# Plachtaa/FAcodec

Hardware: NVIDIA H100
Metric: audio_seconds_per_second (higher is better)
Workload: dtype f32 I/O and accumulation; every product is a 3-MMA split of fp32 operands: fp16 hi + 2^11-scaled fp16 lo (22 mantissa bits, register-promoted accumulation) upstream of the VQ, bf16 hi + bf16 lo (16 bits) downstream

## Files before the change

### facodec_b200/csrc/conv_tc.cu

```cuda
#include <cuda_bf16.h>
#include <cuda_fp16.h>

#include <cstring>
#include <mutex>
#include <type_traits>

#include "common.cuh"
#include "conv_tc_common.cuh"
#include "kernels.h"

namespace fac {

namespace {

using namespace tc;

enum Prec { P_TF32 = 0, P_BF16 = 1, P_F16S = 2, P_F16X2 = 3, P_NONE = -1 };

template <int P> struct PrecT {
    static constexpr int KG = P == P_TF32 ? 4 : 2;
    static constexpr int planes = P == P_F16S ? 1 : 2;
    static constexpr int ksteps = P == P_TF32 ? 2 : 1;
    static constexpr int kind = P == P_TF32 ? WG_TF32 : (P == P_BF16 ? WG_BF16 : WG_F16);
};

__host__ __device__ constexpr int prec_kg(int P) { return P == P_TF32 ? 4 : 2; }
__host__ __device__ constexpr int prec_planes(int P) { return P == P_F16S ? 1 : 2; }
__host__ __device__ constexpr uint32_t master_bytes(bool promoted, int nchunk, int promote_every, int ni) {
    return promoted && nchunk > promote_every ? (uint32_t)ni / 2 * 4 * kThreads : 0u;
}

template <int NI>
__device__ __forceinline__ void zero_acc(float (&a)[NI / 2]) {
#pragma unroll
    for (int i = 0; i < NI / 2; ++i) a[i] = 0.f;
}

template <int P, int NI>
__device__ __forceinline__ void mma_pass(float (&acc)[NI / 2], uint32_t a_addr, uint32_t a_lbo, uint32_t b_addr,
                                         uint32_t b_lbo) {
#pragma unroll
    for (int ks = 0; ks < PrecT<P>::ksteps; ++ks)
        wgmma_ss<NI, PrecT<P>::kind>(acc, gdesc(a_addr + ks * 2 * a_lbo, a_lbo, 128), gdesc(b_addr + ks * 2 * b_lbo, b_lbo, 128));
}

struct Tile {
    int row0, col0, nw;
    int warp, lane;
};

template <int NI, int GROUP = NI, typename F>
__device__ __forceinline__ void for_each_pair(const Tile& tl, const float (&acc)[NI / 2], F&& f) {
#pragma unroll
    for (int j = 0; j < NI / 8; ++j) {
        if (j > 0 && (8 * j) % GROUP == 0 && 8 * j >= tl.nw) break;
#pragma unroll
        for (int h = 0; h < 2; ++h) {
            const int row = tl.row0 + 16 * tl.warp + (tl.lane >> 2) + 8 * h;
            const int col = tl.col0 + 8 * j + 2 * (tl.lane & 3);
            f(row, col, acc[4 * j + 2 * h], acc[4 * j + 2 * h + 1]);
        }
    }
}

template <bool FAST>
__device__ __forceinline__ float act_out(int act, float v, float al, float ia) {
    if (act == ACT_SNAKE) return FAST ? fmaf(ia, sin2_mufu(al * v), v) : snake_fast(v, al, ia);
    if (act == ACT_TANH) return tanhf(v);
    if (act == ACT_MISH) return mish_f(v);
    return v;
}

template <int P1, int P2, bool TT>
constexpr bool groupable() { return P1 != P_F16S && P2 == P_NONE && !TT; }

template <int P1, int P2, bool PROMO, int NI, int MINB, bool TT, bool C2D>
__device__ __forceinline__ void conv_tc_body(const TcConvParams& p) {
    constexpr bool FUSED = P2 != P_NONE;
    constexpr bool GROUPABLE = groupable<P1, P2, TT>() && !C2D;
    static_assert(!C2D || (P1 == P_F16X2 && PROMO && !FUSED && !TT), "2-D taps: the promoted fp16 hi + scaled-lo class only");
    static_assert(!TT || (NI == 64 && !FUSED), "transposed tiles: <= 64 channels x 64 time steps per warpgroup");
    static_assert(NI % 16 == 0 && NI <= (PROMO || MINB == 2 ? 64 : (P1 == P_F16S ? 256 : 128)),
                  "accumulator registers: <= 64 / 128 columns (256 in the one-pass fp16 class at one CTA per SM)");
    constexpr bool F16X2 = P1 == P_F16X2;
    constexpr bool DEC = P1 == P_BF16 || P1 == P_F16S;
    using T1 = PrecT<P1>;
    extern __shared__ __align__(1024) uint8_t smem[];
    uint64_t* full = reinterpret_cast<uint64_t*>(smem);

    const int tid = threadIdx.x, wg = tid >> 7;
    const int BM = 64 * p.MT;
    const int N = p.N, NW = p.MT == 2 ? N : N / 2;
    Tile tl;
    tl.row0 = p.MT == 2 ? 64 * wg : 0;
    tl.col0 = p.MT == 2 ? 0 : wg * NW;
    tl.nw = NW;
    tl.warp = (tid >> 5) & 3;
    tl.lane = tid & 31;
    const int t0 = blockIdx.x * BM, ntile = blockIdx.y, b = blockIdx.z;
    const int Kr = p.Kr, dil = p.dil, Rpad = p.Rpad, nchunk = p.nchunk, S = p.stagesB;
    const int G = GROUPABLE ? p.group : 1;
    const int R = BM + (C2D ? 2 * p.row2d + 2 : (Kr - 1) * dil);
    const int nstep1 = G == 4 ? nchunk >> 2 : (G == 2 ? nchunk >> 1 : nchunk);
    const uint32_t a_plane = (uint32_t)G * T1::KG * Rpad * 16, a_bytes = a_plane * T1::planes;
    uint8_t* abuf = smem + kSmemHdr;
    float4* master = reinterpret_cast<float4*>(abuf + 2 * (size_t)a_bytes);
    const uint32_t m_bytes = master_bytes(PROMO, nchunk, p.promote_every, NI);
    uint8_t* wbuf = abuf + 2 * (size_t)a_bytes + m_bytes;
    uint8_t* a2buf = m_bytes ? reinterpret_cast<uint8_t*>(master) : wbuf + (size_t)S * p.b_slot;
    const uint32_t w_unit1 = (uint32_t)Kr * T1::planes * T1::KG * N * 16;
    const uint32_t w_unit2 = FUSED ? (uint32_t)prec_planes(P2) * prec_kg(P2) * N * 16 : 0;
    const int units = nstep1 + (FUSED ? p.nchunk2 : 0);

    if (tid == 0) {
        for (int i = 0; i < S; ++i) mbar_init(&full[i], 1);
        fence_mbar_init();
    }
    __syncthreads();
    auto issue_w = [&](int u) {
        uint64_t* bar = &full[u % S];
        uint8_t* dst = wbuf + (size_t)(u % S) * p.b_slot;
        const uint8_t* src;
        uint32_t bytes;
        if (u < nstep1) {
            src = reinterpret_cast<const uint8_t*>(p.wblob) + ((size_t)ntile * nchunk + (size_t)u * G) * w_unit1;
            bytes = G * w_unit1;
        } else { src = reinterpret_cast<const uint8_t*>(p.wblob2) + (size_t)(u - nstep1) * w_unit2; bytes = w_unit2; }
        mbar_arrive_expect_tx(bar, bytes);
        bulk_g2s(dst, src, bytes, bar);
    };
    if (tid == 0)
        for (int u = 0; u < S - 1 && u < units; ++u) issue_w(u);

    const PadMap pm = PadMap::lane(p.lane_len, b, p.Tin, p.pad_left_s, p.pad_right_s, p.reflect);
    const float* __restrict__ xb = p.x + (size_t)b * p.x_bstride;
    auto produce = [&](int s) {
        uint8_t* ahi = abuf + (size_t)(s & 1) * a_bytes;
        auto run = [&](auto grouped) {
            constexpr bool GR = decltype(grouped)::value;
            const int c = GR ? s * G : s;
            if constexpr (P1 == P_TF32) produce_chunk<kThreads, GR, false>(p, pm, xb, c, G, t0, R, Rpad, ahi, ahi + a_plane, tid);
            else if constexpr (P1 == P_BF16) produce_chunk<kThreads, GR, true>(p, pm, xb, c, G, t0, R, Rpad, ahi, ahi + a_plane, tid);
            else if constexpr (P1 == P_F16S) produce_chunk<kThreads, GR, true, 4, false, false, true>(p, pm, xb, c, G, t0, R, Rpad, ahi, ahi, tid);
            else produce_chunk<kThreads, GR, false, 4, false, true>(p, pm, xb, c, G, t0, R, Rpad, ahi, ahi + a_plane, tid);
        };
        if constexpr (GROUPABLE) {
            if (G > 1) run(std::true_type());
            else run(std::false_type());
        } else {
            run(std::false_type());
        }
        fence_proxy_async();
    };
    produce(0);

    float acc[NI / 2];
    float crs[F16X2 ? NI / 2 : 1];
    zero_acc<NI>(acc);
    if constexpr (F16X2) zero_acc<NI>(crs);
    const uint32_t a_lbo = (uint32_t)Rpad * 16, b_lbo = (uint32_t)N * 16;
    const uint32_t abase = smem_u32(abuf), wbase = smem_u32(wbuf), a2base = smem_u32(a2buf);
    const int BM2 = BM;

    auto promote = [&](bool first, bool last) {
        if constexpr (PROMO) {
#pragma unroll
            for (int q = 0; q < NI / 8; ++q) {
                float w[4];
#pragma unroll
                for (int e = 0; e < 4; ++e) {
                    const int i = 4 * q + e;
                    if constexpr (F16X2) { w[e] = acc[i] + crs[i] * kLoUnscale; crs[i] = 0.f; }
                    else w[e] = acc[i];
                }
                float4 m = first ? make_float4(0.f, 0.f, 0.f, 0.f) : master[q * kThreads + tid];
                m.x += w[0]; m.y += w[1]; m.z += w[2]; m.w += w[3];
                if (!last) master[q * kThreads + tid] = m;
                acc[4 * q + 0] = last ? m.x : 0.f;
                acc[4 * q + 1] = last ? m.y : 0.f;
                acc[4 * q + 2] = last ? m.z : 0.f;
                acc[4 * q + 3] = last ? m.w : 0.f;
            }
        }
    };

#pragma unroll 1
    for (int u = 0; u < units; ++u) {
        __syncthreads();
        if (tid == 0 && u + S - 1 < units) issue_w(u + S - 1);
        mbar_wait(&full[u % S], (uint32_t)(u / S) & 1u);
        const uint32_t wslot = wbase + (uint32_t)(u % S) * p.b_slot;
        wg_fence();
        if (u < nstep1) {
            const uint32_t a0 = abase + (uint32_t)(u & 1) * a_bytes + (uint32_t)tl.row0 * 16;
            const uint32_t b0 = wslot + (uint32_t)tl.col0 * 16;
            auto mma_tap = [&](uint32_t ahi, uint32_t bhi) {
                const uint32_t alo = ahi + a_plane, blo = bhi + T1::KG * b_lbo;
                if constexpr (TT) {
                    mma_pass<P1, NI>(acc, bhi, b_lbo, ahi, a_lbo);
                    mma_pass<P1, NI>(crs, bhi, b_lbo, alo, a_lbo);
                    mma_pass<P1, NI>(crs, blo, b_lbo, ahi, a_lbo);
                } else if constexpr (P1 == P_F16S) {
                    mma_pass<P1, NI>(acc, ahi, a_lbo, bhi, b_lbo);
                } else if constexpr (F16X2) {
                    mma_pass<P1, NI>(acc, ahi, a_lbo, bhi, b_lbo);
                    mma_pass<P1, NI>(crs, ahi, a_lbo, blo, b_lbo);
                    mma_pass<P1, NI>(crs, alo, a_lbo, bhi, b_lbo);
                } else {
                    mma_pass<P1, NI>(acc, ahi, a_lbo, bhi, b_lbo);
                    mma_pass<P1, NI>(acc, ahi, a_lbo, blo, b_lbo);
// ... 105 lines not shown
    for_each_pair<NI>(tl, acc, [&](int row, int col, float v0, float v1) {
        const int t = t0 + row;
        if (t >= p.Tout) return;
        if constexpr (C2D) {
            const float2 bi = __ldg(reinterpret_cast<const float2*>(bi_p + col));
            v0 += bi.x; v1 += bi.y;
            if (act == ACT_LRELU) { v0 = v0 >= 0.f ? v0 : 0.01f * v0; v1 = v1 >= 0.f ? v1 : 0.01f * v1; }
            if (rb) { const float2 r = *reinterpret_cast<const float2*>(rb + (size_t)t * p.ldy + col); v0 += r.x; v1 += r.y; }
            const int f = t % p.row2d;
            if (f == 0 || f == p.row2d - 1) { v0 = 0.f; v1 = 0.f; }
            *reinterpret_cast<float2*>(yb + (size_t)t * p.ldy + col) = make_float2(v0, v1);
            return;
        }
        if (bi_p) { const float2 bi = __ldg(reinterpret_cast<const float2*>(bi_p + col)); v0 += bi.x; v1 += bi.y; }
        if (act == ACT_SNAKE) {
            const float2 al = __ldg(reinterpret_cast<const float2*>(al_p + col));
            const float2 ia = __ldg(reinterpret_cast<const float2*>(ia_p + col));
            v0 = act_out<DEC>(ACT_SNAKE, v0, al.x, ia.x);
            v1 = act_out<DEC>(ACT_SNAKE, v1, al.y, ia.y);
        } else if (act != ACT_NONE) {
            v0 = act_out<DEC>(act, v0, 0.f, 0.f);
            v1 = act_out<DEC>(act, v1, 0.f, 0.f);
        }
        if (rb) { const float2 r = *reinterpret_cast<const float2*>(rb + (size_t)t * p.ldy + col); v0 += r.x; v1 += r.y; }
        *reinterpret_cast<float2*>(yb + (size_t)t * p.ldy + col) = make_float2(v0, v1);
    });
}

template <int P1, int P2, bool PROMO, int NI, int MINB = 1, bool TT = false>
__global__ void __launch_bounds__(kThreads, groupable<P1, P2, TT>() && NI <= 128 ? 2 : MINB) conv_tc_kernel(TcConvParams p) {
    conv_tc_body<P1, P2, PROMO, NI, MINB, TT, false>(p);
}

template <int NI>
__global__ void __launch_bounds__(kThreads, 2) conv2d_tc_kernel(TcConvParams p) {
    conv_tc_body<P_F16X2, P_NONE, true, NI, 2, false, true>(p);
}

}

namespace {
constexpr size_t kSmemCap = 227 * 1024;
constexpr size_t kSmemCap2 = 113 * 1024;
int plan_prec(const TcConvParams& p) {
    return p.g1f16 ? P_F16S : (p.f16x2 ? P_F16X2 : (p.bf16 ? P_BF16 : P_TF32));
}
constexpr int f16s_wide_nw(bool fused) { return fused ? 192 : 256; }
}

bool tc_conv_plan(TcConvParams& p) {
    if ((p.Cin % 4) != 0 || ((p.Cin * p.vf) % kChunk) != 0 || (p.Cout % 16) != 0) return false;
    if (p.bf16 && p.promoted) return false;
    if (p.f16x2 && !p.promoted) return false;
    if (p.g1f16 && !p.bf16) return false;
    if (p.tt && !p.f16x2) return false;
    if (p.row2d && (p.Kr != 9 || p.vf != 1 || !p.f16x2 || p.tt || p.fused || p.row2d < 3)) return false;
    if (p.fused && ((p.promoted && (!p.f16x2 || p.tt)) || p.Cin != p.Cout || p.vf != 1 || p.Cout > 256)) return false;
    const int P1 = plan_prec(p), P2 = p.fused ? (p.f16x2 ? P_F16X2 : (p.bf16 ? P_BF16 : P_TF32)) : P_NONE;
    p.nchunk = p.Cin * p.vf / kChunk;
    p.nchunk2 = p.fused ? p.Cout / kChunk : 0;
    p.promote_every = p.promoted ? (p.f16x2 ? (48 / p.Kr < 1 ? 1 : 48 / p.Kr) : (8 / p.Kr < 1 ? 1 : 8 / p.Kr)) : 1;
    if (p.fused && p.promoted && p.nchunk2 > 48) return false;
    const int nw_max = p.promoted ? 64 : 128;
    constexpr size_t kAReserve = 40 * 1024;
    int N = 0;
    for (int cand = p.fused ? p.Cout : 256; cand >= 16 && N == 0; cand -= 16) {
// ... 26 lines not shown
        return l;
    };
    auto group = [&](int S, int MT, size_t cap) {
        if (p.Kr > 3 || p.tt || p.fused || p.g1f16) return 1;
        for (int G = 4; G > 1; G /= 2)
            if (G <= p.max_group && p.nchunk % G == 0 && (!p.promoted || p.promote_every % G == 0) && layout(S, MT, G).total <= cap) return G;
        return 1;
    };
    const bool unit2 = p.fused && p.promoted;
    const bool want2 = p.promoted ? !p.tt : (p.occ2_maxn > 0 && N <= p.occ2_maxn);
    for (int two = want2 ? 1 : 0; two >= (unit2 ? 1 : 0); --two) {
        const size_t cap = two ? kSmemCap2 : kSmemCap;
        const int nwl = two ? 64 : nw_max;
        for (int S = 2; S >= 1; --S)
            for (int MT = 2; MT >= 1; --MT) {
                const int NW = MT == 2 ? N : N / 2;
                const bool wide = !two && P1 == P_F16S && NW == f16s_wide_nw(p.fused);
                if ((NW > nwl && !wide) || NW % 16 || (unit2 && NW != 64)) continue;
                if (wide && layout(2, 1, 1).total <= kSmemCap2) continue;
                const Layout l1 = layout(S, MT, 1);
                if (l1.total > cap) continue;
                const int G = group(S, MT, l1.total <= kSmemCap2 ? kSmemCap2 : cap);
                const Layout l = layout(S, MT, G);
                p.N = N; p.MT = MT; p.Rpad = l.Rpad; p.R2pad = 64 * MT; p.stagesB = S; p.b_slot = (int)l.slot;
                p.group = G;
                p.smem_bytes = l.total;
                p.occ2 = two;
                return true;
            }
    }
    return false;
}

size_t tc_blob_floats(const TcConvParams& p) {
    if (p.g1f16) return (size_t)(p.Cout / p.N) * p.nchunk * p.Kr * 2 * p.N * 4;
    return (size_t)(p.Cout / p.N) * p.nchunk * p.Kr * 2 * ((p.bf16 || p.f16x2) ? 2 : 4) * p.N * 4;
}

static inline uint16_t bf16_rn_host(float f) {
    uint32_t u;
    memcpy(&u, &f, 4);
    u += 0x7FFFu + ((u >> 16) & 1u);
    return (uint16_t)(u >> 16);
}

void tc_pack_blob(const TcConvParams& p, const float* wp, int ldw, float* blob) {
    const int Cw = p.Cin * p.vf;
    if (p.g1f16) {
        uint16_t* ob = reinterpret_cast<uint16_t*>(blob);
        size_t o16 = 0;
        for (int nt = 0; nt < p.Cout / p.N; ++nt)
            for (int c = 0; c < p.nchunk; ++c)
                for (int tap = 0; tap < p.Kr; ++tap)
                    for (int k8 = 0; k8 < 2; ++k8)
                        for (int n = 0; n < p.N; ++n)
                            for (int e = 0; e < 8; ++e) {
                                int kk = tap * Cw + c * tc::kChunk + k8 * 8 + e;
                                __half v = __float2half_rn(wp[(size_t)kk * ldw + nt * p.N + n]);
                                uint16_t bits;
                                memcpy(&bits, &v, 2);
                                ob[o16++] = bits;
                            }
        return;
    }
    if (p.f16x2) {
        uint16_t* ob = reinterpret_cast<uint16_t*>(blob);
// ... 31 lines not shown
                                    uint32_t hu = (uint32_t)hi << 16;
                                    float hf;
                                    memcpy(&hf, &hu, 4);
                                    ob[o16++] = hl == 0 ? hi : bf16_rn_host(w - hf);
                                }
        return;
    }
    size_t o = 0;
    for (int nt = 0; nt < p.Cout / p.N; ++nt)
        for (int c = 0; c < p.nchunk; ++c)
            for (int tap = 0; tap < p.Kr; ++tap)
                for (int hl = 0; hl < 2; ++hl)
                    for (int k4 = 0; k4 < 4; ++k4)
                        for (int n = 0; n < p.N; ++n)
                            for (int e = 0; e < 4; ++e) {
                                int kk = tap * Cw + c * tc::kChunk + k4 * 4 + e;
                                float w = wp[(size_t)kk * ldw + nt * p.N + n];
                                uint32_t u;
                                memcpy(&u, &w, 4);
                                uint32_t hu = (u + 0x1000u) & 0xFFFFE000u;
                                float hi;
                                memcpy(&hi, &hu, 4);
                                float lo = w - hi;
                                uint32_t lu;
                                memcpy(&lu, &lo, 4);
                                lu = (lu + 0x1000u) & 0xFFFFE000u;
                                float lo_r;
                                memcpy(&lo_r, &lu, 4);
                                blob[o++] = hl == 0 ? hi : lo_r;
                            }
}

namespace {
template <int P1, int P2, bool PROMO, int NI, int MINB = 1, bool TT = false, bool C2D = false>
cudaError_t launch_one(const TcConvParams& p, dim3 grid, cudaStream_t st) {
    auto* kern = [] {
        if constexpr (C2D) return conv2d_tc_kernel<NI>;
        else return conv_tc_kernel<P1, P2, PROMO, NI, MINB, TT>;
    }();
    static bool done[64] = {};
    static std::mutex mu;
    int dev = 0;
    cudaError_t e = cudaGetDevice(&dev);
    if (e != cudaSuccess) return e;
    if (dev < 0 || dev >= 64) return cudaErrorInvalidDevice;
    {
        std::lock_guard<std::mutex> lk(mu);
        if (!done[dev]) {
            e = cudaFuncSetAttribute(kern, cudaFuncAttributeMaxDynamicSharedMemorySize, (int)kSmemCap);
            if (e != cudaSuccess) return e;
            done[dev] = true;
        }
    }
    kern<<<grid, kThreads, p.smem_bytes, st>>>(p);
    return cudaGetLastError();
}
template <int P1, int P2, bool PROMO, int MINB = 1, int NI = (PROMO || MINB == 2 ? 64 : 128), bool C2D = false>
cudaError_t launch_nw(const TcConvParams& p, dim3 grid, cudaStream_t st) {
    const int NW = p.MT == 2 ? p.N : p.N / 2;
    if (NW == NI) return launch_one<P1, P2, PROMO, NI, MINB, false, C2D>(p, grid, st);
    if constexpr (NI > 16) return launch_nw<P1, P2, PROMO, MINB, NI - 16, C2D>(p, grid, st);
    else return cudaErrorInvalidValue;
}
template <int P1, int P2>
cudaError_t launch_occ(const TcConvParams& p, dim3 grid, cudaStream_t st) {
    if (p.occ2) return launch_nw<P1, P2, false, 2>(p, grid, st);
    if constexpr (P1 == P_F16S) {
        constexpr int kWide = f16s_wide_nw(P2 != P_NONE);
        if ((p.MT == 2 ? p.N : p.N / 2) == kWide) return launch_one<P1, P2, false, kWide>(p, grid, st);
    }
    return launch_nw<P1, P2, false, 1>(p, grid, st);
}
}

cudaError_t launch_conv_tc(const TcConvParams& p, cudaStream_t st) {
    if (p.Tout <= 0 || p.B <= 0) return cudaSuccess;
    const int BM = 64 * p.MT;
    dim3 grid((p.Tout + BM - 1) / BM, p.Cout / p.N, p.B);
    if (grid.y > 65535 || grid.z > 65535) return cudaErrorInvalidValue;
    const int P1 = plan_prec(p);
    if (p.row2d) {
        if (P1 != P_F16X2 || !p.promoted || p.fused || p.tt || p.Kr != 9) return cudaErrorInvalidValue;
        return launch_nw<P_F16X2, P_NONE, true, 2, 64, true>(p, grid, st);
    }
    if (p.fused) {
        if (P1 == P_F16X2)
            return (p.MT == 2 ? p.N : p.N / 2) == 64 ? launch_one<P_F16X2, P_F16X2, true, 64, 2>(p, grid, st) : cudaErrorInvalidValue;
        if (P1 == P_F16S) return launch_occ<P_F16S, P_BF16>(p, grid, st);
        if (P1 == P_BF16) return launch_occ<P_BF16, P_BF16>(p, grid, st);
        return launch_occ<P_TF32, P_TF32>(p, grid, st);
    }
    if (p.tt) return launch_one<P_F16X2, P_NONE, true, 64, 1, true>(p, grid, st);
    if (p.promoted)
        return P1 == P_F16X2 ? launch_nw<P_F16X2, P_NONE, true, 2>(p, grid, st) : launch_nw<P_TF32, P_NONE, true, 2>(p, grid, st);
    if (P1 == P_F16S) return launch_occ<P_F16S, P_NONE>(p, grid, st);
    if (P1 == P_BF16) return launch_occ<P_BF16, P_NONE>(p, grid, st);
    return launch_occ<P_TF32, P_NONE>(p, grid, st);
}

}
```

### facodec_b200/csrc/engine.cu

```cuda
#include <cmath>
#include <cstddef>
#include <cstdio>
#include <cstdlib>
#include <cstring>
#include <algorithm>
#include <initializer_list>
#include <map>
#include <memory>
#include <string>
#include <type_traits>
#include <vector>

#include "../../include/facodec_b200.h"
#include "../../include/facodec_b200_debug.h"
#include "common.cuh"
#include "kernels.h"
#include "resample.h"

using namespace fac;

namespace {

constexpr int HOP = 300;
constexpr int LATENT = 1024;
// ... 652 lines not shown

int conv_out_len(int T, int k_eff, int stride) {
    int padding_total = k_eff - stride;
    double n_frames = (double)(T - k_eff + padding_total) / stride + 1.0;
    int ideal = ((int)std::ceil(n_frames) - 1) * stride + (k_eff - padding_total);
    int extra = ideal - T;
    return (T + padding_total + extra - k_eff) / stride + 1;
}
int conv_extra_pad(int T, int k_eff, int stride) {
    int padding_total = k_eff - stride;
    double n_frames = (double)(T - k_eff + padding_total) / stride + 1.0;
    int ideal = ((int)std::ceil(n_frames) - 1) * stride + (k_eff - padding_total);
    return ideal - T;
}

void run_conv(Ctx& c, const ConvW& w, const float* x, float* y, int B, int Tin, int Tout, const ConvOpts& o,
              const char* name) {
    if (c.dry) return;
    if (c.h->use_tc >= (c.vq_critical ? 2 : 1) && w.tc && !o.transposed && !o.valid_len && (o.ldx == 0 || o.ldx == w.Cin) &&
        (o.ldy == 0 || o.ldy == w.Cout) && o.stride == w.vf && (w.vf == 1 || o.dil == 1) && !o.no_bias) {
        TcConvParams tp;
        tp.Cin = w.Cin; tp.Cout = w.Cout; tp.vf = w.vf; tp.Kr = w.Kr; tp.promoted = w.promoted ? 1 : 0;
        tp.dil = w.vf == 1 ? o.dil : 1;
        tp.bf16 = (c.h->dec_bf16 && w.has16 && !w.promoted && !c.vq_critical) ? 1 : 0;
        tp.g1f16 = (tp.bf16 && w.has_f16s && c.h->dec_c7_f16) ? 1 : 0;
        tp.f16x2 = (tp.promoted && c.h->enc_f16 && w.has16) ? 1 : 0;
        tp.occ2_maxn = c.h->tc_occ2;
        tp.Tout = Tout;
        if (tp.f16x2 && c.h->enc_tt) {
            TcConvParams t2 = tp;
            t2.tt = 1;
            if (tc_conv_plan(t2)) tp = t2;
        }
        if (tc_conv_plan(tp)) {
            tp.x = x; tp.y = y; tp.wblob = c.W(tp.g1f16 ? w.tcw_f16s : ((tp.bf16 || tp.f16x2) ? w.tcw16 : w.tcw)); tp.bias = c.W(w.b);
            if (o.in_snake) { tp.in_alpha = c.W(o.in_snake->a); tp.in_inv_alpha = c.W(o.in_snake->ia); }
            tp.out_act = o.act;
            if (o.out_snake) { tp.out_act = ACT_SNAKE; tp.out_alpha = c.W(o.out_snake->a); tp.out_inv_alpha = c.W(o.out_snake->ia); }
            tp.res = o.res;
            tp.B = B; tp.Tin = Tin; tp.ldx = w.Cin;
            tp.PLr = o.pad_left / w.vf;
            tp.pad_left_s = o.pad_left; tp.pad_right_s = o.pad_right; tp.reflect = o.reflect; tp.lane_len = o.lane_len;
            tp.Tout = Tout; tp.ldy = w.Cout;
            tp.x_bstride = (size_t)Tin * w.Cin; tp.y_bstride = (size_t)Tout * w.Cout;
            double flops = 2.0 * B * Tout * (double)w.Cout * w.K * w.Cin;
            double bytes = 4.0 * ((double)B * Tin * w.Cin + (double)B * Tout * w.Cout * (o.res ? 2 : 1) + (double)w.K * w.Cin * w.Cout);
            char det[96];
            snprintf(det, sizeof det, "%s Cin%d Cout%d K%d d%d T%d", name, w.Cin, w.Cout, w.K, o.dil, Tout);
            c.begin(tp.promoted ? "conv_tcp" : "conv_tc", flops, bytes, det);
            c.check(launch_conv_tc(tp, c.st), name);
            c.end();
            return;
        }
    }
    ConvParams p;
    p.x = x; p.y = y;
    p.w = c.W(w.w);
    p.bias = o.no_bias ? nullptr : c.W(w.b);
    if (o.in_snake) { p.in_alpha = c.W(o.in_snake->a); p.in_inv_alpha = c.W(o.in_snake->ia); }
    p.out_act = o.act;
    if (o.out_snake) { p.out_act = ACT_SNAKE; p.out_alpha = c.W(o.out_snake->a); p.out_inv_alpha = c.W(o.out_snake->ia); }
    p.res = o.res; p.valid_len = o.valid_len; p.lane_len = o.lane_len;
    p.B = B; p.Tin = Tin; p.Cin = w.Cin; p.Tout = Tout; p.Cout = w.Cout;
    p.K = w.K; p.dil = o.dil; p.stride = o.stride;
    p.pad_left = o.pad_left; p.pad_right = o.pad_right; p.pad_reflect = o.reflect;
    p.ldw = w.ldw; p.ldy = o.ldy ? o.ldy : w.Cout; p.ldx = o.ldx ? o.ldx : w.Cin;
    p.y_transposed = o.transposed;
// ... 12 lines not shown
          const char* name, bool causal = true) {
    int k_eff = (w.K - 1) * dil + 1;
    o.dil = dil; o.stride = stride;
    const int total = k_eff - stride, extra = conv_extra_pad(T, k_eff, stride);
    o.pad_left = causal ? total : total - total / 2;
    o.pad_right = (causal ? 0 : total / 2) + extra;
    o.reflect = 1;
    int Tout = conv_out_len(T, k_eff, stride);
    run_conv(c, w, x, y, B, T, Tout, o, name);
    return Tout;
}

bool residual_unit_fused(Ctx& c, const ResW& r, const float* x, float* y, int B, int T, bool causal, const int* lane_len) {
    const bool promoted = r.c7.promoted && r.c1.promoted;
    if (!c.h->fuse_res || !r.c7.tc || !r.c1.tc || r.c7.promoted != r.c1.promoted || r.c7.Cin != r.c7.Cout ||
        r.c1.K != 1 || r.c7.vf != 1)
        return false;
    if (c.vq_critical ? (!promoted || c.h->use_tc < 2 || !c.h->enc_f16 || c.h->enc_tt || !r.c7.has16 || !r.c1.has16)
                      : (promoted || c.h->use_tc < 1))
        return false;
    TcConvParams tp;
    tp.Cin = r.c7.Cin; tp.Cout = r.c7.Cout; tp.vf = 1; tp.Kr = r.c7.K; tp.dil = r.dil; tp.fused = 1;
    tp.promoted = promoted ? 1 : 0;
    tp.f16x2 = tp.promoted;
    tp.bf16 = (!promoted && c.h->dec_bf16 && r.c7.has16 && r.c1.has16) ? 1 : 0;
    tp.g1f16 = (tp.bf16 && r.c7.has_f16s && c.h->dec_c7_f16) ? 1 : 0;
    tp.occ2_maxn = c.h->tc_occ2;
    tp.Tout = T;
    if (c.h->fuse_res == 2 && r.c7.Cout > 128) return false;
    if (!tc_conv_plan(tp)) return false;
    TcConvParams q7 = tp, q1 = tp;
    q7.fused = 0; q1.fused = 0; q1.Kr = 1; q1.g1f16 = 0;
    if (!tc_conv_plan(q7) || !tc_conv_plan(q1) || q7.N != tp.N || q1.N != tp.N) return false;
    if (c.dry) return true;
    const int k_eff = (r.c7.K - 1) * r.dil + 1;
    tp.x = x; tp.y = y; tp.res = x;
    tp.wblob = c.W(tp.g1f16 ? r.c7.tcw_f16s : ((tp.bf16 || tp.f16x2) ? r.c7.tcw16 : r.c7.tcw)); tp.bias = c.W(r.c7.b);
    tp.wblob2 = c.W((tp.bf16 || tp.f16x2) ? r.c1.tcw16 : r.c1.tcw); tp.bias2 = c.W(r.c1.b);
    tp.in_alpha = c.W(r.s1.a); tp.in_inv_alpha = c.W(r.s1.ia);
    tp.out_act = ACT_SNAKE; tp.out_alpha = c.W(r.s2.a); tp.out_inv_alpha = c.W(r.s2.ia);
    tp.B = B; tp.Tin = T; tp.ldx = r.c7.Cin;
    const int pl = causal ? k_eff - 1 : (k_eff - 1) - (k_eff - 1) / 2;
    tp.PLr = pl; tp.pad_left_s = pl; tp.pad_right_s = k_eff - 1 - pl; tp.reflect = 1; tp.lane_len = lane_len;
    tp.Tout = T; tp.ldy = r.c7.Cout;
    tp.x_bstride = (size_t)T * r.c7.Cin; tp.y_bstride = (size_t)T * r.c7.Cout;
    double flops = 2.0 * B * T * (double)r.c7.Cout * r.c7.Cin * (r.c7.K + 1);
    double bytes = 4.0 * ((double)B * T * r.c7.Cin * 2 + (double)B * T * r.c7.Cout + (double)(r.c7.K + 1) * r.c7.Cin * r.c7.Cout);
    char det[96];
    snprintf(det, sizeof det, "res.fused C%d K%d d%d T%d", r.c7.Cin, r.c7.K, r.dil, T);
    c.begin(tp.promoted ? "conv_tcp" : "conv_tc", flops, bytes, det);
    c.check(launch_conv_tc(tp, c.st), "res.fused");
    c.end();
    return true;
}

void residual_unit(Ctx& c, const ResW& r, const float* x, float* tmp, float* y, int B, int T, bool causal = true,
                   const int* lane_len = nullptr) {
    if (residual_unit_fused(c, r, x, y, B, T, causal, lane_len)) return;
    ConvOpts o1;
    o1.in_snake = &r.s1;
    o1.out_snake = &r.s2;
    o1.lane_len = lane_len;
    sconv(c, r.c7, x, tmp, B, T, r.dil, 1, o1, "res.conv7", causal);
    ConvOpts o2;
    o2.res = x;
    sconv(c, r.c1, tmp, y, B, T, 1, 1, o2, "res.conv1", causal);
// ... 3681 lines not shown
    cudaSetDevice(h->device);
    cudaStream_t st = (cudaStream_t)stream;
    cudaError_t e = launch_attention(q, k, v, o, B, T, heads, 256, valid_len, st, force_stream ? 1 : 0);
    if (e == cudaSuccess) e = cudaStreamSynchronize(st);
    if (e != cudaSuccess) { h->err = std::string("fac_debug_attention: ") + cudaGetErrorString(e); return FAC_ERR_CUDA; }
    return FAC_OK;
}

int fac_set_option(fac_handle* h, const char* name, int value) {
    if (!h || !name) return FAC_ERR_INVALID;
    if (std::string(name) == "fuse_resunit") { h->fuse_res = value < 0 ? 0 : (value > 2 ? 2 : value); return FAC_OK; }
    if (std::string(name) == "encoder_f16x2") { h->enc_f16 = value != 0; return FAC_OK; }
    if (std::string(name) == "encoder_tt") { h->enc_tt = value != 0; return FAC_OK; }
    if (std::string(name) == "tc_occ2_maxn") { h->tc_occ2 = value < 0 ? 0 : value; return FAC_OK; }
    if (std::string(name) == "decoder_conv7_fp16") { h->dec_c7_f16 = value != 0; return FAC_OK; }
    if (std::string(name) == "overlap_front") { h->overlap_front = value != 0; return FAC_OK; }
    if (std::string(name) == "lstm_v2") { h->lstm_v2 = value != 0; return FAC_OK; }
    if (std::string(name) == "decoder_lstm_fp16") { h->dec_lstm_fp16 = value != 0; return FAC_OK; }
    if (std::string(name) == "attention_stream") { h->attn_stream = value != 0; return FAC_OK; }
    if (std::string(name) == "decoder_bf16") { h->dec_bf16 = value != 0; return FAC_OK; }
    if (std::string(name) == "tensor_cores") { h->use_tc = value < 0 ? 0 : (value > 2 ? 2 : value); return FAC_OK; }
    h->err = std::string("unknown option ") + name;
    return FAC_ERR_INVALID;
}

static int debug_conv_tc(fac_handle* h, const float* x, const float* w_host, const float* bias_host, int B, int Tin, int Cin,
                         int Cout, int K, int dil, int stride, int pad_left, int pad_right, int reflect,
                         const float* in_alpha_host, const float* out_alpha_host, int act, const float* res, float* y,
                         int Tout, int promoted, void* stream, int* group_out, const int* lane_len) {
    if (!h || !x || !w_host || !y) return FAC_ERR_INVALID;
    cudaSetDevice(h->device);
    cudaStream_t st = (cudaStream_t)stream;
    TcConvParams tp;
    tp.Cin = Cin; tp.Cout = Cout; tp.promoted = (promoted == 1 || promoted == 3 || promoted == 4) ? 1 : 0;
    tp.bf16 = (promoted == 2 || promoted == 5) ? 1 : 0;
    tp.f16x2 = (promoted == 3 || promoted == 4) ? 1 : 0;
    tp.tt = promoted == 4 ? 1 : 0;
    tp.g1f16 = promoted == 5 ? 1 : 0;
    tp.occ2_maxn = h->tc_occ2;
    tp.Tout = Tout;
    if (stride == 1) { tp.vf = 1; tp.Kr = K; tp.dil = dil; }
    else if (K == 2 * stride && dil == 1) { tp.vf = stride; tp.Kr = 2; tp.dil = 1; }
    else { h->err = "fac_debug_conv_tc: unsupported stride/kernel"; return FAC_ERR_UNSUPPORTED; }
    if (promoted < 0 || promoted > 5 || !tc_conv_plan(tp)) { h->err = "fac_debug_conv_tc: layer not eligible for the tensor-core path"; return FAC_ERR_UNSUPPORTED; }
    if (group_out) {
        *group_out = tp.group;
        tp.max_group = 1;
        if (!tc_conv_plan(tp)) { h->err = "fac_debug_conv_tc_group1: no one-chunk plan"; return FAC_ERR_UNSUPPORTED; }
    }
    int ldw = (Cout + 3) / 4 * 4;
    std::vector<float> gen((size_t)K * Cin * ldw, 0.f);
    for (int co = 0; co < Cout; ++co)
        for (int ci = 0; ci < Cin; ++ci)
            for (int k = 0; k < K; ++k) gen[((size_t)k * Cin + ci) * ldw + co] = w_host[((size_t)co * Cin + ci) * K + k];
    size_t nb = tc_blob_floats(tp);
    auto al4 = [](size_t v) { return (v + 3) / 4 * 4; };
    size_t o_b = al4(nb), o_ia = al4(o_b + Cout), o_iia = al4(o_ia + Cin), o_oa = al4(o_iia + Cin), o_oia = al4(o_oa + Cout);
    std::vector<float> pk(o_oia + Cout + 16, 0.f);
    tc_pack_blob(tp, gen.data(), ldw, pk.data());
    for (int i = 0; i < Cout; ++i) pk[o_b + i] = bias_host ? bias_host[i] : 0.f;
    for (int i = 0; i < Cin; ++i) { pk[o_ia + i] = in_alpha_host ? in_alpha_host[i] : 1.f; pk[o_iia + i] = 1.0f / (pk[o_ia + i] + 1e-9f); }
    for (int i = 0; i < Cout; ++i) { pk[o_oa + i] = out_alpha_host ? out_alpha_host[i] : 1.f; pk[o_oia + i] = 1.0f / (pk[o_oa + i] + 1e-9f); }
    DevBuf<float> buf;
    const int rc = upload(h, pk, buf, "fac_debug_conv_tc");
    if (rc != FAC_OK) return rc;
    const float* d = buf.get();
    tp.x = x; tp.y = y; tp.wblob = d; tp.bias = d + o_b;
    if (in_alpha_host) { tp.in_alpha = d + o_ia; tp.in_inv_alpha = d + o_iia; }
    tp.out_act = act;
    if (out_alpha_host) { tp.out_act = ACT_SNAKE; tp.out_alpha = d + o_oa; tp.out_inv_alpha = d + o_oia; }
    tp.res = res;
    tp.B = B; tp.Tin = Tin; tp.ldx = Cin;
    tp.PLr = pad_left / tp.vf;
    tp.pad_left_s = pad_left; tp.pad_right_s = pad_right; tp.reflect = reflect; tp.lane_len = lane_len;
    tp.Tout = Tout; tp.ldy = Cout;
    tp.x_bstride = (size_t)Tin * Cin; tp.y_bstride = (size_t)Tout * Cout;
    cudaError_t e = launch_conv_tc(tp, st);
    if (e == cudaSuccess) e = cudaStreamSynchronize(st);
    if (e != cudaSuccess) { h->err = std::string("fac_debug_conv_tc: ") + cudaGetErrorString(e); return FAC_ERR_CUDA; }
    return FAC_OK;
}
// ... 130 lines not shown
    ts["c.weight"] = std::move(t);
    ts["c.bias"] = std::move(b);
    Packer P;
    ConvW c;
    try { c = causal ? pack_convtr(P, ts, "c", stride) : pack_convtr_noncausal(P, ts, "c", stride); }
    catch (const PackError&) { return FAC_ERR_UNSUPPORTED; }
    const long long n = (long long)c.K * Cin * c.Cout;
    if (!out || capacity_floats < n) return n;
    for (int k = 0; k < c.K; ++k)
        for (int ci = 0; ci < Cin; ++ci)
            for (int co = 0; co < c.Cout; ++co) out[((size_t)k * Cin + ci) * c.Cout + co] = P.pack[c.w + ((size_t)k * Cin + ci) * c.ldw + co];
    return n;
}

int fac_debug_pad_map(int L, int pad_left, int pad_right, int reflect, int* out, int n) {
    if (!out || L < 0 || pad_left < 0 || pad_right < 0 || n != pad_left + L + pad_right) return FAC_ERR_INVALID;
    const PadMap pm = PadMap::make(L, pad_left, pad_right, reflect);
    for (int i = 0; i < n; ++i) out[i] = pm.src(i - pad_left);
    return FAC_OK;
}

int fac_debug_lane_pad_map(const int* lane_len, int B, int Tin, int pad_left, int pad_right, int reflect, int* out, int n) {
    if (!out || B <= 0 || Tin < 0 || pad_left < 0 || pad_right < 0 || n != pad_left + Tin + pad_right) return FAC_ERR_INVALID;
    for (int b = 0; lane_len && b < B; ++b)
        if (lane_len[b] < 0 || lane_len[b] > Tin) return FAC_ERR_INVALID;
    for (int b = 0; b < B; ++b) {
        const PadMap pm = PadMap::lane(lane_len, b, Tin, pad_left, pad_right, reflect);
        for (int i = 0; i < n; ++i) out[(size_t)b * n + i] = pm.src(i - pad_left);
    }
    return FAC_OK;
}

static int debug_tc_plan(int Cin, int Cout, int K, int dil, int stride, int Tout, int mode, int occ2_maxn, TcConvParams& tp) {
    if (Cin <= 0 || Cout <= 0 || K <= 0 || dil <= 0 || stride <= 0 || mode < 0 || mode > 9) return FAC_ERR_INVALID;
    tp.Cin = Cin; tp.Cout = Cout; tp.Tout = Tout; tp.occ2_maxn = occ2_maxn;
    tp.promoted = (mode == 1 || mode == 3 || mode == 9) ? 1 : 0;
    tp.bf16 = (mode == 2 || mode == 4 || mode == 7 || mode == 8) ? 1 : 0;
    tp.f16x2 = (mode == 3 || mode == 9) ? 1 : 0;
    tp.fused = (mode == 4 || mode == 5 || mode == 8 || mode == 9) ? 1 : 0;
    tp.g1f16 = (mode == 7 || mode == 8) ? 1 : 0;
    if (mode == 6) { tp.promoted = 1; tp.f16x2 = 1; tp.tt = 1; }
    if (stride == 1) { tp.vf = 1; tp.Kr = K; tp.dil = dil; }
    else if (K == 2 * stride && dil == 1) { tp.vf = stride; tp.Kr = 2; tp.dil = 1; }
    else return FAC_ERR_UNSUPPORTED;
    return tc_conv_plan(tp) ? FAC_OK : FAC_ERR_UNSUPPORTED;
}

int fac_debug_tc_plan(int Cin, int Cout, int K, int dil, int stride, int Tout, int mode, int occ2_maxn, int* out8) {
    if (!out8) return FAC_ERR_INVALID;
    TcConvParams tp;
    const int rc = debug_tc_plan(Cin, Cout, K, dil, stride, Tout, mode, occ2_maxn, tp);
    if (rc != FAC_OK) return rc;
    out8[0] = tp.N; out8[1] = tp.MT; out8[2] = tp.nchunk; out8[3] = tp.stagesB; out8[4] = tp.R2pad;
    out8[5] = (int)tp.smem_bytes; out8[6] = tp.Rpad; out8[7] = tp.promote_every;
    return FAC_OK;
}

int fac_debug_tc_plan_group(int Cin, int Cout, int K, int dil, int stride, int Tout, int mode, int occ2_maxn, int* smem2) {
    TcConvParams tp;
    const int rc = debug_tc_plan(Cin, Cout, K, dil, stride, Tout, mode, occ2_maxn, tp);
    if (rc != FAC_OK) return rc;
    if (smem2) {
        TcConvParams t1 = tp;
        t1.max_group = 1;
        if (!tc_conv_plan(t1)) return FAC_ERR_UNSUPPORTED;
        smem2[0] = (int)tp.smem_bytes;
        smem2[1] = (int)t1.smem_bytes;
    }
    return tp.group;
}

long long fac_debug_tc_pack(const float* w_host, int Cin, int Cout, int K, int stride, int mode, float* blob_out,
                            long long capacity_floats) {
    if (!w_host || Cin <= 0 || Cout <= 0 || K <= 0 || stride <= 0 || mode < 0 || mode > 3) return FAC_ERR_INVALID;
    TcConvParams tp;
    tp.Cin = Cin; tp.Cout = Cout; tp.dil = 1;
    tp.promoted = (mode == 1 || mode == 3) ? 1 : 0; tp.bf16 = mode == 2 ? 1 : 0; tp.f16x2 = mode == 3 ? 1 : 0;
    if (stride == 1) { tp.vf = 1; tp.Kr = K; }
// ... 115 lines not shown
```

### facodec_b200/csrc/kernels.h

```cpp
#pragma once
#include <cuda_runtime.h>
#include <stdint.h>

namespace fac {

struct ConvParams {
    const float* x = nullptr;
    const float* w = nullptr;
    const float* bias = nullptr;
    const float* in_alpha = nullptr;
    const float* in_inv_alpha = nullptr;
    const float* out_alpha = nullptr;
    const float* out_inv_alpha = nullptr;
    const float* res = nullptr;
    const int* valid_len = nullptr;
    const int* lane_len = nullptr;
    float* y = nullptr;
    int B = 0, Tin = 0, Cin = 0, Tout = 0, Cout = 0;
    int K = 1, dil = 1, stride = 1, pad_left = 0, pad_right = 0, pad_reflect = 0;
    int ldw = 0, ldy = 0, ldx = 0;
    int out_act = 0;
    int y_transposed = 0;
    size_t x_bstride = 0, y_bstride = 0;
};
// ... 7 lines not shown
    const float* in_inv_alpha = nullptr;
    const float* out_alpha = nullptr;
    const float* out_inv_alpha = nullptr;
    const float* res = nullptr;
    float* y = nullptr;
    int B = 0, Tin = 0, Cin = 0, ldx = 0;
    int vf = 1;
    int Kr = 1, dil = 1, PLr = 0;
    int pad_left_s = 0, pad_right_s = 0, reflect = 0;
    const int* lane_len = nullptr;
    int Tout = 0, Cout = 0, ldy = 0;
    int out_act = 0;
    int promoted = 0;
    int bf16 = 0;
    int g1f16 = 0;
    int f16x2 = 0;
    int fused = 0;
    int tt = 0;
    int occ2_maxn = 0;
    int max_group = 4;
    const float* wblob2 = nullptr;
    const float* bias2 = nullptr;
    int nchunk2 = 0;
    int promote_every = 1;
    int N = 0, nchunk = 0, Rpad = 0, stagesB = 0;
    int group = 1;
    int MT = 2;
    int b_slot = 0;
    int occ2 = 0;
    int R2pad = 0;
    size_t smem_bytes = 0;
    size_t x_bstride = 0, y_bstride = 0;
    int row2d = 0;
};
bool tc_conv_plan(TcConvParams& p);
size_t tc_blob_floats(const TcConvParams& p);
void tc_pack_blob(const TcConvParams& p, const float* wp, int ldw, float* blob);
cudaError_t launch_conv_tc(const TcConvParams& p, cudaStream_t st);

struct LstmParams {
    const float* xg = nullptr;
    const float* whh_p = nullptr;
    const float* whh_p16 = nullptr;
    int bf16 = 0;
    const uint32_t* whh_p2 = nullptr;
    uint32_t* h16 = nullptr;
    int pass3 = 0;
    uint32_t* state_h = nullptr;
    float* state_c = nullptr;
    const float* skip = nullptr;
    float* y = nullptr;
    float* hT = nullptr;
    unsigned int* bar = nullptr;
    int B = 0, T = 0, H = 0, U = 0, G = 0;
};
struct LstmLaneLens { int len[32]; };
cudaError_t launch_lstm_layer(const LstmParams& p, cudaStream_t st);
cudaError_t launch_lstm2_layer(const LstmParams& p, cudaStream_t st, const LstmLaneLens* lens = nullptr, bool reverse = false);
size_t lstm2_pack_words(int H, int U, int pass3);
void lstm2_pack(const float* whh, int H, int U, int pass3, uint32_t* out);
size_t lstm2_smem_bytes(int H, int U, int pass3);
void lstm2_state_sizes(int H, int U, int pass3, size_t* h_words, size_t* c_floats);
cudaError_t lstm2_read_phase_clocks(long long* out4);
void lstm2_lane_map(int H, int U, int pass3, int b, long long* pos);
constexpr int kLaneMax = 32;
struct LaneCarryParams {
    uint32_t* slot[kLaneMax];
    uint32_t* state_h = nullptr;
// ... 126 lines not shown
```

Baseline: 1052.

## Add four-warpgroup wide kernel for promoted fp16x2 K=7 convs at N=128

New measurement: 1069 (median of 6 runs). 1.02x the previous value.

```diff
diff --git a/facodec_b200/csrc/conv_tc.cu b/facodec_b200/csrc/conv_tc.cu
--- a/facodec_b200/csrc/conv_tc.cu
+++ b/facodec_b200/csrc/conv_tc.cu
@@ -26,9 +26,10 @@
 
 __host__ __device__ constexpr int prec_kg(int P) { return P == P_TF32 ? 4 : 2; }
 __host__ __device__ constexpr int prec_planes(int P) { return P == P_F16S ? 1 : 2; }
-__host__ __device__ constexpr uint32_t master_bytes(bool promoted, int nchunk, int promote_every, int ni) {
-    return promoted && nchunk > promote_every ? (uint32_t)ni / 2 * 4 * kThreads : 0u;
-}
+__host__ __device__ constexpr uint32_t master_bytes(bool promoted, int nchunk, int promote_every, int ni, int threads = kThreads) {
+    return promoted && nchunk > promote_every ? (uint32_t)ni / 2 * 4 * threads : 0u;
+}
+constexpr int kWideThreads = 4 * 128;
 
 template <int NI>
 __device__ __forceinline__ void zero_acc(float (&a)[NI / 2]) {
@@ -74,9 +75,12 @@
 template <int P1, int P2, bool TT>
 constexpr bool groupable() { return P1 != P_F16S && P2 == P_NONE && !TT; }
 
-template <int P1, int P2, bool PROMO, int NI, int MINB, bool TT, bool C2D>
+template <int P1, int P2, bool PROMO, int NI, int MINB, bool TT, bool C2D, int NT = kThreads>
 __device__ __forceinline__ void conv_tc_body(const TcConvParams& p) {
     constexpr bool FUSED = P2 != P_NONE;
+    constexpr bool WIDE = NT == kWideThreads;
+    static_assert(NT == kThreads || (WIDE && P1 == P_F16X2 && PROMO && NI == 64 && !TT && !C2D),
+                  "four warpgroups: the promoted fp16 hi + scaled-lo class at 64 channels per warpgroup only");
     constexpr bool GROUPABLE = groupable<P1, P2, TT>() && !C2D;
     static_assert(!C2D || (P1 == P_F16X2 && PROMO && !FUSED && !TT), "2-D taps: the promoted fp16 hi + scaled-lo class only");
     static_assert(!TT || (NI == 64 && !FUSED), "transposed tiles: <= 64 channels x 64 time steps per warpgroup");
@@ -90,10 +94,10 @@
 
     const int tid = threadIdx.x, wg = tid >> 7;
     const int BM = 64 * p.MT;
-    const int N = p.N, NW = p.MT == 2 ? N : N / 2;
+    const int N = p.N, NW = WIDE ? N / 2 : (p.MT == 2 ? N : N / 2);
     Tile tl;
-    tl.row0 = p.MT == 2 ? 64 * wg : 0;
-    tl.col0 = p.MT == 2 ? 0 : wg * NW;
+    tl.row0 = WIDE ? 64 * (wg & 1) : (p.MT == 2 ? 64 * wg : 0);
+    tl.col0 = WIDE ? (wg >> 1) * NW : (p.MT == 2 ? 0 : wg * NW);
     tl.nw = NW;
     tl.warp = (tid >> 5) & 3;
     tl.lane = tid & 31;
@@ -105,7 +109,7 @@
     const uint32_t a_plane = (uint32_t)G * T1::KG * Rpad * 16, a_bytes = a_plane * T1::planes;
     uint8_t* abuf = smem + kSmemHdr;
     float4* master = reinterpret_cast<float4*>(abuf + 2 * (size_t)a_bytes);
-    const uint32_t m_bytes = master_bytes(PROMO, nchunk, p.promote_every, NI);
+    const uint32_t m_bytes = master_bytes(PROMO, nchunk, p.promote_every, NI, NT);
     uint8_t* wbuf = abuf + 2 * (size_t)a_bytes + m_bytes;
     uint8_t* a2buf = m_bytes ? reinterpret_cast<uint8_t*>(master) : wbuf + (size_t)S * p.b_slot;
     const uint32_t w_unit1 = (uint32_t)Kr * T1::planes * T1::KG * N * 16;
@@ -139,10 +143,10 @@
         auto run = [&](auto grouped) {
             constexpr bool GR = decltype(grouped)::value;
             const int c = GR ? s * G : s;
-            if constexpr (P1 == P_TF32) produce_chunk<kThreads, GR, false>(p, pm, xb, c, G, t0, R, Rpad, ahi, ahi + a_plane, tid);
-            else if constexpr (P1 == P_BF16) produce_chunk<kThreads, GR, true>(p, pm, xb, c, G, t0, R, Rpad, ahi, ahi + a_plane, tid);
-            else if constexpr (P1 == P_F16S) produce_chunk<kThreads, GR, true, 4, false, false, true>(p, pm, xb, c, G, t0, R, Rpad, ahi, ahi, tid);
-            else produce_chunk<kThreads, GR, false, 4, false, true>(p, pm, xb, c, G, t0, R, Rpad, ahi, ahi + a_plane, tid);
+            if constexpr (P1 == P_TF32) produce_chunk<NT, GR, false>(p, pm, xb, c, G, t0, R, Rpad, ahi, ahi + a_plane, tid);
+            else if constexpr (P1 == P_BF16) produce_chunk<NT, GR, true>(p, pm, xb, c, G, t0, R, Rpad, ahi, ahi + a_plane, tid);
+            else if constexpr (P1 == P_F16S) produce_chunk<NT, GR, true, 4, false, false, true>(p, pm, xb, c, G, t0, R, Rpad, ahi, ahi, tid);
+            else produce_chunk<NT, GR, false, 4, false, true>(p, pm, xb, c, G, t0, R, Rpad, ahi, ahi + a_plane, tid);
         };
         if constexpr (GROUPABLE) {
             if (G > 1) run(std::true_type());
@@ -173,9 +177,9 @@
                     if constexpr (F16X2) { w[e] = acc[i] + crs[i] * kLoUnscale; crs[i] = 0.f; }
                     else w[e] = acc[i];
                 }
-                float4 m = first ? make_float4(0.f, 0.f, 0.f, 0.f) : master[q * kThreads + tid];
+                float4 m = first ? make_float4(0.f, 0.f, 0.f, 0.f) : master[q * NT + tid];
                 m.x += w[0]; m.y += w[1]; m.z += w[2]; m.w += w[3];
-                if (!last) master[q * kThreads + tid] = m;
+                if (!last) master[q * NT + tid] = m;
                 acc[4 * q + 0] = last ? m.x : 0.f;
                 acc[4 * q + 1] = last ? m.y : 0.f;
                 acc[4 * q + 2] = last ? m.z : 0.f;
@@ -347,6 +351,11 @@
     conv_tc_body<P1, P2, PROMO, NI, MINB, TT, false>(p);
 }
 
+template <int P2>
+__global__ void __launch_bounds__(kWideThreads, 1) conv_tcp_wide_kernel(TcConvParams p) {
+    conv_tc_body<P_F16X2, P2, true, 64, 1, false, false, kWideThreads>(p);
+}
+
 template <int NI>
 __global__ void __launch_bounds__(kThreads, 2) conv2d_tc_kernel(TcConvParams p) {
     conv_tc_body<P_F16X2, P_NONE, true, NI, 2, false, true>(p);
@@ -439,6 +448,23 @@
     return false;
 }
 
+bool tc_conv_plan_promoted_wide(TcConvParams& p) {
+    if (!p.promoted || !p.f16x2 || p.tt || p.row2d || p.vf != 1 || p.Kr != 7) return false;
+    TcConvParams q = p;
+    if (!tc_conv_plan(q) || q.N != 128) return false;
+    constexpr int BM = 128, S = 2, kPieces = 2 * 2;
+    int Rpad = BM + (q.Kr - 1) * q.dil;
+    while (Rpad % 8 != 2) ++Rpad;
+    const size_t a_bytes = (size_t)kPieces * Rpad * 16, slot = (size_t)q.Kr * kPieces * q.N * 16;
+    const size_t master = master_bytes(true, q.nchunk, q.promote_every, q.N / 2, kWideThreads);
+    const size_t total = kSmemHdr + 2 * a_bytes + master + S * slot;
+    if (total > kSmemCap || (q.fused && (size_t)kPieces * q.nchunk2 * BM * 16 > master)) return false;
+    q.MT = 2; q.Rpad = Rpad; q.R2pad = BM; q.stagesB = S; q.b_slot = (int)slot; q.group = 1;
+    q.smem_bytes = total; q.occ2 = 0; q.wide = 1;
+    p = q;
+    return true;
+}
+
 size_t tc_blob_floats(const TcConvParams& p) {
     if (p.g1f16) return (size_t)(p.Cout / p.N) * p.nchunk * p.Kr * 2 * p.N * 4;
     return (size_t)(p.Cout / p.N) * p.nchunk * p.Kr * 2 * ((p.bf16 || p.f16x2) ? 2 : 4) * p.N * 4;
@@ -536,10 +562,11 @@
 }
 
 namespace {
-template <int P1, int P2, bool PROMO, int NI, int MINB = 1, bool TT = false, bool C2D = false>
+template <int P1, int P2, bool PROMO, int NI, int MINB = 1, bool TT = false, bool C2D = false, bool WIDE = false>
 cudaError_t launch_one(const TcConvParams& p, dim3 grid, cudaStream_t st) {
     auto* kern = [] {
         if constexpr (C2D) return conv2d_tc_kernel<NI>;
+        else if constexpr (WIDE) return conv_tcp_wide_kernel<P2>;
         else return conv_tc_kernel<P1, P2, PROMO, NI, MINB, TT>;
     }();
     static bool done[64] = {};
@@ -556,7 +583,7 @@
             done[dev] = true;
         }
     }
-    kern<<<grid, kThreads, p.smem_bytes, st>>>(p);
+    kern<<<grid, WIDE ? kWideThreads : kThreads, p.smem_bytes, st>>>(p);
     return cudaGetLastError();
 }
 template <int P1, int P2, bool PROMO, int MINB = 1, int NI = (PROMO || MINB == 2 ? 64 : 128), bool C2D = false>
@@ -583,6 +610,11 @@
     dim3 grid((p.Tout + BM - 1) / BM, p.Cout / p.N, p.B);
     if (grid.y > 65535 || grid.z > 65535) return cudaErrorInvalidValue;
     const int P1 = plan_prec(p);
+    if (p.wide) {
+        if (P1 != P_F16X2 || !p.promoted || p.tt || p.MT != 2 || p.N != 128) return cudaErrorInvalidValue;
+        return p.fused ? launch_one<P_F16X2, P_F16X2, true, 64, 1, false, false, true>(p, grid, st)
+                       : launch_one<P_F16X2, P_NONE, true, 64, 1, false, false, true>(p, grid, st);
+    }
     if (p.row2d) {
         if (P1 != P_F16X2 || !p.promoted || p.fused || p.tt || p.Kr != 9) return cudaErrorInvalidValue;
         return launch_nw<P_F16X2, P_NONE, true, 2, 64, true>(p, grid, st);
diff --git a/facodec_b200/csrc/engine.cu b/facodec_b200/csrc/engine.cu
--- a/facodec_b200/csrc/engine.cu
+++ b/facodec_b200/csrc/engine.cu
@@ -708,7 +708,7 @@
             t2.tt = 1;
             if (tc_conv_plan(t2)) tp = t2;
         }
-        if (tc_conv_plan(tp)) {
+        if ((tp.f16x2 && !tp.tt && tc_conv_plan_promoted_wide(tp)) || tc_conv_plan(tp)) {
             tp.x = x; tp.y = y; tp.wblob = c.W(tp.g1f16 ? w.tcw_f16s : ((tp.bf16 || tp.f16x2) ? w.tcw16 : w.tcw)); tp.bias = c.W(w.b);
             if (o.in_snake) { tp.in_alpha = c.W(o.in_snake->a); tp.in_inv_alpha = c.W(o.in_snake->ia); }
             tp.out_act = o.act;
@@ -787,6 +787,7 @@
     TcConvParams q7 = tp, q1 = tp;
     q7.fused = 0; q1.fused = 0; q1.Kr = 1; q1.g1f16 = 0;
     if (!tc_conv_plan(q7) || !tc_conv_plan(q1) || q7.N != tp.N || q1.N != tp.N) return false;
+    if (tp.promoted) tc_conv_plan_promoted_wide(tp);
     if (c.dry) return true;
     const int k_eff = (r.c7.K - 1) * r.dil + 1;
     tp.x = x; tp.y = y; tp.res = x;
@@ -4534,9 +4535,9 @@
     cudaSetDevice(h->device);
     cudaStream_t st = (cudaStream_t)stream;
     TcConvParams tp;
-    tp.Cin = Cin; tp.Cout = Cout; tp.promoted = (promoted == 1 || promoted == 3 || promoted == 4) ? 1 : 0;
+    tp.Cin = Cin; tp.Cout = Cout; tp.promoted = (promoted == 1 || promoted == 3 || promoted == 4 || promoted == 6) ? 1 : 0;
     tp.bf16 = (promoted == 2 || promoted == 5) ? 1 : 0;
-    tp.f16x2 = (promoted == 3 || promoted == 4) ? 1 : 0;
+    tp.f16x2 = (promoted == 3 || promoted == 4 || promoted == 6) ? 1 : 0;
     tp.tt = promoted == 4 ? 1 : 0;
     tp.g1f16 = promoted == 5 ? 1 : 0;
     tp.occ2_maxn = h->tc_occ2;
@@ -4544,11 +4545,17 @@
     if (stride == 1) { tp.vf = 1; tp.Kr = K; tp.dil = dil; }
     else if (K == 2 * stride && dil == 1) { tp.vf = stride; tp.Kr = 2; tp.dil = 1; }
     else { h->err = "fac_debug_conv_tc: unsupported stride/kernel"; return FAC_ERR_UNSUPPORTED; }
-    if (promoted < 0 || promoted > 5 || !tc_conv_plan(tp)) { h->err = "fac_debug_conv_tc: layer not eligible for the tensor-core path"; return FAC_ERR_UNSUPPORTED; }
+    if (promoted < 0 || promoted > 6 || !(promoted == 6 ? tc_conv_plan_promoted_wide(tp) : tc_conv_plan(tp))) {
+        h->err = "fac_debug_conv_tc: layer not eligible for the tensor-core path";
+        return FAC_ERR_UNSUPPORTED;
+    }
     if (group_out) {
         *group_out = tp.group;
         tp.max_group = 1;
-        if (!tc_conv_plan(tp)) { h->err = "fac_debug_conv_tc_group1: no one-chunk plan"; return FAC_ERR_UNSUPPORTED; }
+        if (!(promoted == 6 ? tc_conv_plan_promoted_wide(tp) : tc_conv_plan(tp))) {
+            h->err = "fac_debug_conv_tc_group1: no one-chunk plan";
+            return FAC_ERR_UNSUPPORTED;
+        }
     }
     int ldw = (Cout + 3) / 4 * 4;
     std::vector<float> gen((size_t)K * Cin * ldw, 0.f);
@@ -4745,18 +4752,18 @@
 }
 
 static int debug_tc_plan(int Cin, int Cout, int K, int dil, int stride, int Tout, int mode, int occ2_maxn, TcConvParams& tp) {
-    if (Cin <= 0 || Cout <= 0 || K <= 0 || dil <= 0 || stride <= 0 || mode < 0 || mode > 9) return FAC_ERR_INVALID;
+    if (Cin <= 0 || Cout <= 0 || K <= 0 || dil <= 0 || stride <= 0 || mode < 0 || mode > 10) return FAC_ERR_INVALID;
     tp.Cin = Cin; tp.Cout = Cout; tp.Tout = Tout; tp.occ2_maxn = occ2_maxn;
-    tp.promoted = (mode == 1 || mode == 3 || mode == 9) ? 1 : 0;
+    tp.promoted = (mode == 1 || mode == 3 || mode == 9 || mode == 10) ? 1 : 0;
     tp.bf16 = (mode == 2 || mode == 4 || mode == 7 || mode == 8) ? 1 : 0;
-    tp.f16x2 = (mode == 3 || mode == 9) ? 1 : 0;
+    tp.f16x2 = (mode == 3 || mode == 9 || mode == 10) ? 1 : 0;
     tp.fused = (mode == 4 || mode == 5 || mode == 8 || mode == 9) ? 1 : 0;
     tp.g1f16 = (mode == 7 || mode == 8) ? 1 : 0;
     if (mode == 6) { tp.promoted = 1; tp.f16x2 = 1; tp.tt = 1; }
     if (stride == 1) { tp.vf = 1; tp.Kr = K; tp.dil = dil; }
     else if (K == 2 * stride && dil == 1) { tp.vf = stride; tp.Kr = 2; tp.dil = 1; }
     else return FAC_ERR_UNSUPPORTED;
-    return tc_conv_plan(tp) ? FAC_OK : FAC_ERR_UNSUPPORTED;
+    return (mode == 10 ? tc_conv_plan_promoted_wide(tp) : tc_conv_plan(tp)) ? FAC_OK : FAC_ERR_UNSUPPORTED;
 }
 
 int fac_debug_tc_plan(int Cin, int Cout, int K, int dil, int stride, int Tout, int mode, int occ2_maxn, int* out8) {
diff --git a/facodec_b200/csrc/kernels.h b/facodec_b200/csrc/kernels.h
--- a/facodec_b200/csrc/kernels.h
+++ b/facodec_b200/csrc/kernels.h
@@ -63,8 +63,10 @@
     size_t smem_bytes = 0;
     size_t x_bstride = 0, y_bstride = 0;
     int row2d = 0;
+    int wide = 0;
 };
 bool tc_conv_plan(TcConvParams& p);
+bool tc_conv_plan_promoted_wide(TcConvParams& p);
 size_t tc_blob_floats(const TcConvParams& p);
 void tc_pack_blob(const TcConvParams& p, const float* wp, int ldw, float* blob);
 cudaError_t launch_conv_tc(const TcConvParams& p, cudaStream_t st);
```
